# PJLab-ADG/neuralsim

Hardware: NVIDIA H100
Metric: Mrays/sec fwd+bwd (higher is better)
Workload: dtype f16

## Files before the change

### neuralsim_b200/csrc/color_tc.cu

```cuda
#include "fused_tc_common.cuh"
#include "sh_device.cuh"

namespace nsb {

struct ColorNetDev {
    DecoderDevTC dec;
    const __half *R1, *rb1, *R2, *rb2, *R3, *rb3;
    int rw, rin, n_appear;
    float fac[3];
};

constexpr int XW = 64;
constexpr int kTileBytes = kTile * XW * 2;
constexpr int kChunk = kTile * 16;

__host__ __device__ inline int ref_col(int k, int n_appear, int nh) {
    if (k < 32) return k < nh ? 22 + k : -1;
    if (k < 35) return k - 32;
    if (k < 51) return 3 + (k - 35);
    if (k < 54) return 19 + (k - 51);
    if (k < 54 + n_appear) return 22 + nh + (k - 54);
    return -1;
}

// ... 388 lines not shown
        __syncthreads();
        if (tid == 0 && tile + gridDim.x < n_tiles) {
            tc::fence_async_smem();
            fetch(tile + gridDim.x);
        }
#pragma unroll
        for (int h = 0; h < 2; ++h)
#pragma unroll
            for (int r = 0; r < 2; ++r) {
                const int64_t row = tile * kTile + h * 64 + tc::frag_row(r);
                if (row < n) {
#pragma unroll
                    for (int c = 0; c < NF / 8; ++c)
                        *reinterpret_cast<float2 *>(dh_out + row * NF + tc::frag_col(c)) = make_float2(dh[h][4 * c + 2 * r], dh[h][4 * c + 2 * r + 1]);
                    if constexpr (kAppear) *reinterpret_cast<float2 *>(da_out + row * 8 + tc::frag_col(0)) = make_float2(da[h][2 * r], da[h][2 * r + 1]);
                    if constexpr (kRays) {
#pragma unroll
                        for (int c = 0; c < 3; ++c)
                            *reinterpret_cast<float2 *>(xv_out + row * 24 + tc::frag_col(c)) = make_float2(dxv[h][4 * c + 2 * r], dxv[h][4 * c + 2 * r + 1]);
                    }
                }
            }
    }
    if (!first_tile) {
#pragma unroll
        for (int r = 0; r < 2; ++r) {
            const int row = tc::frag_row(r);
            if (row >= net.rw) continue;
#pragma unroll
            for (int c = 0; c < NE / 8; ++c)
#pragma unroll
                for (int j = 0; j < 2; ++j) {
                    const int col = tc::frag_col(c) + j;
                    const float a = xa[4 * c + 2 * r + j], b = xb[4 * c + 2 * r + j];
                    if (col < XW) {
                        if (col < net.rw) atomicAdd(dR2 + row * net.rw + col, a);
                        const int rc = ref_col(col, net.n_appear, net.dec.nh);
                        if (rc >= 0) atomicAdd(dR1 + row * net.rin + rc, b);
                    } else if (col == XW) {
                        atomicAdd(drb2 + row, a);
                        atomicAdd(drb1 + row, b);
                    }
                }
#pragma unroll
            for (int j = 0; j < 2; ++j) {
                const int col = tc::frag_col(0) + j;
                if (col >= 1 && col <= 3) atomicAdd(dR3 + (col - 1) * net.rw + row, x3[2 * r + j]);
            }
        }
        if (tid < 3) atomicAdd(drb3 + tid, sdb3[tid]);
    }
}

template <bool kXGrad>
__global__ void __launch_bounds__(kTile, kColorBwdCtasPerSM)
k_color_sdf_bwd(const PLMeta m, const __half *__restrict__ grid, const ColorNetDev net, const PointSrc ps, const uint8_t *__restrict__ Zt,
                const uint8_t *__restrict__ Xt, const float *__restrict__ g_nab, const float *__restrict__ g_sdf, const float *__restrict__ dh_r,
                int64_t n, int max_level, float *__restrict__ d_grid, float *__restrict__ d_W1, float *__restrict__ d_b1, float *__restrict__ d_W2,
                float *__restrict__ d_b2, const int64_t *__restrict__ n_dev, const float *__restrict__ xv_rows,
                const float *__restrict__ view_dirs, float *__restrict__ gx_out) {
    n = eff_n(n, n_dev);
    constexpr int NX = 48;
    extern __shared__ uint8_t dyn_smem[];
    uint8_t *tiles = reinterpret_cast<uint8_t *>((reinterpret_cast<uintptr_t>(dyn_smem) + 1023) & ~uintptr_t(1023));
    uint8_t *sT = tiles;
    uint8_t *sHe = sT + 3 * kTileBytes;
    uint8_t *sGe = sHe + kTile * NX * 2;
    uint8_t *sW1 = sGe + kTile * NX * 2;
    uint8_t *sW1T = sW1 + HW * NF * 2;
    uint8_t *sZ = sW1T + NF * HW * 2;
    constexpr int kS = tc::acc_stride(2 * NF);
    float *stage = reinterpret_cast<float *>(sT);
    static_assert(kTile * kS * 4 <= 3 * kTileBytes, "the staged rows must fit in T");
    __shared__ float sW2[HW], sdsdf[kTile];
    __shared__ float sdb2;
    __shared__ __align__(8) uint64_t mbar_ld;

    const int tid = threadIdx.x, lane = tid & 31;
    stage_W1(net.dec, sW1, tid);
    stage_W1T(net.dec, sW1T, tid);
    stage_decoder_vectors(net.dec, nullptr, sW2, nullptr, tid);
    *reinterpret_cast<uint4 *>(sHe + 4 * kChunk + tid * 16) = make_uint4(0x00003C00u, 0, 0, 0);
    *reinterpret_cast<uint4 *>(sGe + 4 * kChunk + tid * 16) = make_uint4(0x00003C00u, 0, 0, 0);
    *reinterpret_cast<uint4 *>(sHe + 5 * kChunk + tid * 16) = make_uint4(0, 0, 0, 0);
    *reinterpret_cast<uint4 *>(sGe + 5 * kChunk + tid * 16) = make_uint4(0, 0, 0, 0);
    float wacc[NX / 2], vacc[4];
#pragma unroll
    for (int k = 0; k < NX / 2; ++k) wacc[k] = 0.f;
#pragma unroll
    for (int k = 0; k < 4; ++k) vacc[k] = 0.f;
    if (tid == 0) {
        sdb2 = 0.f;
        tc::mbar_init(&mbar_ld, 1);
        tc::fence_mbar_init();
    }
    tc::fence_async_smem();
    __syncthreads();
    const uint32_t t_addr = tc::smem_u32(sT), he_addr = tc::smem_u32(sHe), ge_addr = tc::smem_u32(sGe), w1_addr = tc::smem_u32(sW1),
                   w1t_addr = tc::smem_u32(sW1T);
    const SoftplusK spk(net.dec.beta);
    uint32_t ld_phase = 0;
    bool first_tile = true;

    const int64_t n_tiles = (n + kTile - 1) / kTile;
    auto fetch = [&](int64_t tile) {
        tc::mbar_arrive_expect_tx(&mbar_ld, kTileBytes + 4 * kChunk);
        tc::tma_load_bulk(sZ, Zt + tile * kTileBytes, kTileBytes, &mbar_ld);
        tc::tma_load_bulk(sHe, Xt + tile * kTileBytes, 4 * kChunk, &mbar_ld);
    };
    if (tid == 0 && (int64_t)blockIdx.x < n_tiles) fetch(blockIdx.x);
    for (int64_t tile = blockIdx.x; tile < n_tiles; tile += gridDim.x) {
        const int64_t i = tile * kTile + tid;
        const bool valid = i < n;
        float xn[3], xs[3];
        int64_t ray;
        load_point(ps, ps.x == nullptr, i, valid, xn, xs, ray);
        float gin[3] = {0.f, 0.f, 0.f};
        if (valid && g_nab) {
#pragma unroll
            for (int d = 0; d < 3; ++d) gin[d] = g_nab[i * 3 + d] * net.fac[d] * 0.5f;
        }
        const float dsdf = (valid && g_sdf) ? g_sdf[i] : 0.f;
        sdsdf[tid] = dsdf;
        tc::mbar_wait(&mbar_ld, ld_phase);
        ld_phase ^= 1;
#pragma unroll 1
        for (int c = 0; c < 8; ++c) {
            float z[8], uu[8];
            unpack8(*reinterpret_cast<const uint4 *>(sZ + c * kChunk + tid * 16), z);
#pragma unroll
            for (int j = 0; j < 8; ++j) {
                float a, s;
                softplus_as(z[j], spk, a, s);
                uu[j] = sW2[c * 8 + j] * s;
            }
            *reinterpret_cast<uint4 *>(sT + kTileBytes + c * kChunk + tid * 16) = tc::pack8_f16(uu);
        }
#pragma unroll 4
        for (uint32_t p = 0; p < 16; ++p) {
            uint32_t packed = 0;
            if (p < m.n_pseudo && (int)m.level[p] <= max_level) {
                float J0[3], J1[3];
                level_jacobian(m, p, xs, grid, J0, J1);
                float a0 = 0.f, a1 = 0.f;
#pragma unroll
                for (int d = 0; d < 3; ++d) { a0 = __fmaf_rn(gin[d], J0[d], a0); a1 = __fmaf_rn(gin[d], J1[d], a1); }
                const __half2 h = __floats2half2_rn(a0, a1);
                packed = *reinterpret_cast<const uint32_t *>(&h);
            }
            *reinterpret_cast<uint32_t *>(sGe + (p >> 2) * kChunk + tid * 16 + (p & 3) * 4) = packed;
        }
        tc::fence_async_smem();
        __syncthreads();
        float gfr[2][NF / 2];
        {
            float du[2][HW / 2];
            tc::mma_m128<64, 0, 0, NF / 16>(du, tc::kmajor(ge_addr, kTile), tc::kmajor(w1_addr, HW), false);
            tc::mma_m128<32, 0, 0, HW / 16>(gfr, tc::kmajor(t_addr + kTileBytes, kTile), tc::kmajor(w1t_addr, NF), false);
#pragma unroll
            for (int h = 0; h < 2; ++h)
#pragma unroll
                for (int r = 0; r < 2; ++r) {
                    const int row = h * 64 + tc::frag_row(r);
                    const float ds = sdsdf[row];
#pragma unroll
                    for (int c = 0; c < HW / 8; ++c) {
                        const int col = tc::frag_col(c);
                        const uint32_t off = tc::pair_off<kTile>(row, col);
                        const float2 z2 = tc::ld_pair_f16(sZ, off);
                        float dz[2], vv[2];
#pragma unroll
                        for (int j = 0; j < 2; ++j) {
                            const float z = j ? z2.y : z2.x;
                            float a, s;
                            softplus_as(z, spk, a, s);
                            const float w2 = sW2[col + j], d = r16(du[h][4 * c + 2 * r + j]);
                            const float curv = (z * spk.k > spk.thr) ? 0.f : spk.beta * s * (1.f - s);
                            dz[j] = d * w2 * curv + ds * w2 * s;
                            vv[j] = d * s + ds * r16(a);
                        }
                        tc::st_pair_f16(sT, off, dz[0], dz[1]);
                        tc::st_pair_f16(sT + 2 * kTileBytes, off, vv[0], vv[1]);
                    }
                }
        }
        tc::fence_async_smem();
        __syncthreads();
        float dhz[2][NF / 2];
        tc::mma_m128<32, 0, 0, HW / 16>(dhz, tc::kmajor(t_addr, kTile), tc::kmajor(w1t_addr, NF), false);
        tc::mma_m64<NX, 1, 1, kTile / 16>(wacc, tc::mnmajor(t_addr, kTile), tc::mnmajor(he_addr, kTile), true);
        tc::mma_m64<NF, 1, 1, kTile / 16>(*reinterpret_cast<float(*)[NF / 2]>(wacc), tc::mnmajor(t_addr + kTileBytes, kTile), tc::mnmajor(ge_addr, kTile), true);
        tc::mma_m64<8, 1, 1, kTile / 16>(vacc, tc::mnmajor(t_addr + 2 * kTileBytes, kTile), tc::mnmajor(ge_addr + 4 * kChunk, kTile), true);
        first_tile = false;
        const float dsum = warp_sum(dsdf);
        if (lane == 0 && dsum != 0.f) atomicAdd(&sdb2, dsum);
        __syncthreads();
        if (tid == 0 && tile + gridDim.x < n_tiles) {
            tc::fence_async_smem();
            fetch(tile + gridDim.x);
        }
        tc::frag_store<NF>(gfr, stage, kS, 0);
        tc::frag_store<NF>(dhz, stage, kS, NF);
        __syncthreads();
        float gx[3] = {0.f, 0.f, 0.f};
#pragma unroll 1
        for (uint32_t g4 = 0; g4 * 4 < m.n_pseudo; ++g4) {
            float gg[8], hz[8];
            tc::acc_ld8(stage, kS, tid, g4 * 8, gg);
            tc::acc_ld8(stage, kS, tid, NF + g4 * 8, hz);
            if (valid && dh_r) {
                const float4 r0 = *reinterpret_cast<const float4 *>(dh_r + i * NF + g4 * 8), r1 = *reinterpret_cast<const float4 *>(dh_r + i * NF + g4 * 8 + 4);
                hz[0] += r0.x; hz[1] += r0.y; hz[2] += r0.z; hz[3] += r0.w; hz[4] += r1.x; hz[5] += r1.y; hz[6] += r1.z; hz[7] += r1.w;
            }
#pragma unroll
            for (uint32_t q = 0; q < 4; ++q) {
                const uint32_t p = g4 * 4 + q;
                if (p >= m.n_pseudo || (int)m.level[p] > max_level) continue;
                uint32_t cell[8];
                float w[8], fr[3], sc[3], ua[8], ub[8];
                level_cells3(m, p, xs, cell, w, fr, sc);
                const float g0 = valid ? r16(gg[2 * q]) : 0.f, g1 = valid ? r16(gg[2 * q + 1]) : 0.f;
                const float h0 = valid ? hz[2 * q] : 0.f, h1 = valid ? hz[2 * q + 1] : 0.f;
                if constexpr (kXGrad) level_input_grad(m, p, grid, cell, fr, sc, h0, h1, gx);
#pragma unroll
                for (int c = 0; c < 8; ++c) {
                    float wsum = 0.f;
#pragma unroll
                    for (int gd = 0; gd < 3; ++gd) {
                        float ww = __fmul_rn(sc[gd], gin[gd]);
#pragma unroll
                        for (int d = 0; d < 3; ++d) {
                            if (d == gd) continue;
                            ww = __fmul_rn(ww, (c & (1 << d)) ? fr[d] : __fsub_rn(1.f, fr[d]));
                        }
                        wsum += (c & (1 << gd)) ? ww : -ww;
                    }
                    ua[c] = g0 * wsum + h0 * w[c];
                    ub[c] = g1 * wsum + h1 * w[c];
                }
                if (warp_merge_updates(cell_key3(m, p, xs), valid, ua, ub, lane)) {
                    float2 *gp = level_grad_ptr(m, p, d_grid);
#pragma unroll
                    for (int c = 0; c < 8; ++c) red_add2(gp + cell[c], ua[c], ub[c]);
                }
            }
        }
        if constexpr (kXGrad) {
            if (valid) {
                float g[3], gv[3] = {0.f, 0.f, 0.f};
#pragma unroll
                for (int d = 0; d < 3; ++d) g[d] = input_grad_to_net(gx[d]);
                if (xv_rows) {
                    const float *xr = xv_rows + i * 24;
#pragma unroll
                    for (int d = 0; d < 3; ++d) g[d] = __fadd_rn(g[d], xr[d]);
                    float jx[16], jy[16], jz[16];
                    sh_jacobian(view_dirs[ray * 3], view_dirs[ray * 3 + 1], view_dirs[ray * 3 + 2], 4, jx, jy, jz);
#pragma unroll
                    for (int c = 0; c < 16; ++c) {
                        const float dsh = xr[3 + c];
                        gv[0] = fmaf(dsh, jx[c], gv[0]); gv[1] = fmaf(dsh, jy[c], gv[1]); gv[2] = fmaf(dsh, jz[c], gv[2]);
                    }
                }
                const float tt = ps.t[i];
                float4 *o = reinterpret_cast<float4 *>(gx_out + i * 12);
                o[0] = make_float4(g[0], g[1], g[2], __fmul_rn(tt, g[0]));
                o[1] = make_float4(__fmul_rn(tt, g[1]), __fmul_rn(tt, g[2]), gv[0], gv[1]);
                o[2] = make_float4(gv[2], 0.f, 0.f, 0.f);
            }
        }
        __syncthreads();
    }
    if (!first_tile) {
#pragma unroll
        for (int r = 0; r < 2; ++r) {
            const int row = tc::frag_row(r);
            if (row >= net.dec.width) continue;
#pragma unroll
            for (int c = 0; c <= NF / 8; ++c)
#pragma unroll
                for (int j = 0; j < 2; ++j) {
                    const int col = tc::frag_col(c) + j;
                    if (col < net.dec.nh) atomicAdd(d_W1 + row * net.dec.nh + col, wacc[4 * c + 2 * r + j]);
                    else if (col == NF) atomicAdd(d_b1 + row, wacc[4 * c + 2 * r + j]);
                }
            if (tc::frag_col(0) == 0) atomicAdd(d_W2 + row, vacc[2 * r]);
        }
        if (tid == 0) atomicAdd(d_b2, sdb2);
    }
}

}

using namespace nsb;

namespace {
int make_net(const nsb_color_net *c, const nsb_lotd_meta *meta, PLMeta *m, ColorNetDev *d, const char *who, bool radiance) {
    const nsb_sdf_decoder dec{c->W1, c->b1, c->W2, c->b2, c->width, c->beta};
    if (int rc = make_decoder(meta, &dec, m, &d->dec, who)) return rc;
    if (radiance || c->rad_width != 0) {
        NSB_REQUIRE(c->rad_width >= 1 && c->rad_width <= 64, "%s: radiance width must be <= 64", who);
        NSB_REQUIRE(c->n_appear >= 0 && c->n_appear <= 8 && c->rad_in == 22 + d->dec.nh + c->n_appear,
                    "%s: radiance input must be [x(3), SH deg 4 (16), n(3), h(2L = %d), h_appear(<=8)]", who, d->dec.nh);
    } else {
        NSB_REQUIRE(!c->R1 && !c->rb1 && !c->R2 && !c->rb2 && !c->R3 && !c->rb3, "%s: rad_width 0 (no radiance net) needs NULL radiance pointers", who);
    }
    d->R1 = (const __half *)c->R1; d->rb1 = (const __half *)c->rb1; d->R2 = (const __half *)c->R2; d->rb2 = (const __half *)c->rb2;
    d->R3 = (const __half *)c->R3; d->rb3 = (const __half *)c->rb3;
    d->rw = c->rad_width; d->rin = c->rad_in; d->n_appear = c->n_appear;
    for (int k = 0; k < 3; ++k) d->fac[k] = c->nablas_scale[k];
    return 0;
}
}

static int64_t n_tiles(int64_t n) { return (n + kTile - 1) / kTile; }

extern "C" int64_t nsb_color_tile_bytes(int64_t n) { return n_tiles(n) * (int64_t)kTileBytes; }

extern "C" int nsb_fused_color_fwd(const nsb_lotd_meta *meta, const void *params_half, const nsb_color_net *net, const float *x, const float *rays_o,
                                   const float *rays_d, const int64_t *ridx, const float *t, const float *view_dirs, const float *h_appear,
                                   int64_t n, int32_t max_level, float *sdf, float *nablas, float *rgb, float *x_out, void *act_z, void *act_x,
                                   void *act_y1, void *act_y2, const nsb_occ_collect *collect, void *stream) {
    const DevCounts dn = take_counts();
    if (n == 0) return 0;
    const bool rad = rgb != nullptr;
// ... 25 lines not shown
    constexpr int kSmem = 2 * kTileBytes + 2 * HW * NF * 2 + 2 * XW * XW * 2 + kTile * tc::acc_stride(64) * 4 + 1024;
    opt_in_smem(k_color_fwd<true>, kSmem);
    k_color_fwd<true><<<persistent_grid(n_tiles(n), 2), kTile, kSmem, (cudaStream_t)stream>>>(m, (const __half *)params_half, d, ps, view_dirs, h_appear, n,
                                                                                             ml, sdf, nablas, rgb, x_out, (uint8_t *)act_z,
                                                                                             (uint8_t *)act_x, (uint8_t *)act_y1, (uint8_t *)act_y2,
                                                                                             occ_collect_of(collect), dn.a);
    return check_launch("nsb_fused_color_fwd");
}

template <bool kAppear, bool kRays>
static int color_bwd(const char *who, const nsb_lotd_meta *meta, const void *params_half, const nsb_color_net *net, const float *x, const float *rays_o,
                     const float *rays_d, const int64_t *ridx, const float *t, int64_t n, int32_t max_level, const void *act_z, const void *act_x,
                     const void *act_y1, const void *act_y2, const float *rgb, const float *g_sdf, const float *g_nablas, const float *g_rgb,
                     float *dh_scratch, float *d_grid, float *d_W1, float *d_b1, float *d_W2, float *d_b2, float *d_R1, float *d_rb1, float *d_R2,
                     float *d_rb2, float *d_R3, float *d_rb3, const float *view_dirs, float *ha_scratch, const int64_t *ray_map, float *d_h_appear,
                     float *ray_scratch, float *d_rays_o, float *d_rays_d, float *d_view_dirs, void *stream) {
    const DevCounts dn = take_counts();
    if (n == 0) return 0;
    NSB_REQUIRE(meta && params_half && net && act_z && act_x, "%s: NULL argument", who);
    NSB_REQUIRE(d_grid && d_W1 && d_b1 && d_W2 && d_b2, "%s: NULL gradient buffer", who);
    if (g_rgb) {
        NSB_REQUIRE(act_y1 && act_y2 && rgb && dh_scratch, "%s: NULL argument (g_rgb given)", who);
        NSB_REQUIRE(d_R1 && d_rb1 && d_R2 && d_rb2 && d_R3 && d_rb3, "%s: NULL radiance gradient buffer (g_rgb given)", who);
    }
    if (kAppear) NSB_REQUIRE(g_rgb && ha_scratch && d_h_appear, "%s: needs g_rgb, ha_scratch and d_h_appear", who);
    if (kRays) {
        NSB_REQUIRE(!x && rays_o && rays_d && t && ray_scratch, "%s: ray gradients need the points as rays (x NULL, rays_o, rays_d, t) and ray_scratch", who);
        NSB_REQUIRE(!g_rgb || view_dirs, "%s: ray gradients with g_rgb need view_dirs", who);
    }
    NSB_REQUIRE(x || (rays_o && rays_d && t), "%s: need x or (rays_o, rays_d, t)", who);
    PLMeta m;
    ColorNetDev d;
    if (int rc = make_net(net, meta, &m, &d, who, g_rgb != nullptr)) return rc;
    if (kAppear) NSB_REQUIRE(d.n_appear >= 1, "%s: the net has no appearance channels", who);
    cudaStream_t s = (cudaStream_t)stream;
    const float *dh = nullptr;
    float *xv_rows = (kRays && g_rgb) ? ray_scratch + n * 12 : nullptr;
    if (g_rgb) {
        constexpr int kSmemR = 3 * kTileBytes + 2 * kTile * 80 * 2 + XW * XW * 2 + NF * XW * 2 + (kAppear || kRays ? 8 * XW * 2 : 0) +
                               (kRays ? NF * XW * 2 : 0) + 1024;
        opt_in_smem(k_color_rad_bwd<kAppear, kRays>, kSmemR);
        if (int rc = require_ctas_per_sm(k_color_rad_bwd<kAppear, kRays>, kTile, kSmemR, kColorBwdCtasPerSM, "nsb_fused_color_bwd(radiance)")) return rc;
        k_color_rad_bwd<kAppear, kRays><<<persistent_grid(n_tiles(n), kColorBwdCtasPerSM), kTile, kSmemR, s>>>(
            d, (const uint8_t *)act_x, (const uint8_t *)act_y1, (const uint8_t *)act_y2, rgb, g_rgb, n, dh_scratch, d_R1, d_rb1, d_R2, d_rb2, d_R3, d_rb3,
            dn.a, ha_scratch, xv_rows);
        if (int rc = check_launch("nsb_fused_color_bwd(radiance)")) return rc;
        dh = dh_scratch;
        if (kAppear) {
            k_ray_row_sum<8><<<row_sum_blocks(n), 256, 0, s>>>(ha_scratch, ridx, nullptr, n, d.n_appear, ray_map,
                                                                RowSumOut{{d_h_appear, nullptr, nullptr}, d.n_appear}, dn.a);
            if (int rc = check_launch("nsb_fused_color_bwd(code sum)")) return rc;
        }
    }
    constexpr int kSmemS = 3 * kTileBytes + 2 * kTile * 48 * 2 + 2 * HW * NF * 2 + kTileBytes + 1024;
    opt_in_smem(k_color_sdf_bwd<kRays>, kSmemS);
    if (int rc = require_ctas_per_sm(k_color_sdf_bwd<kRays>, kTile, kSmemS, kColorBwdCtasPerSM, "nsb_fused_color_bwd(sdf)")) return rc;
    const PointSrc ps{x, rays_o, rays_d, t, ridx};
    k_color_sdf_bwd<kRays><<<persistent_grid(n_tiles(n), kColorBwdCtasPerSM), kTile, kSmemS, s>>>(
        m, (const __half *)params_half, d, ps, (const uint8_t *)act_z, (const uint8_t *)act_x, g_nablas, g_sdf, dh, n, max_level < 0 ? -1 : max_level,
        d_grid, d_W1, d_b1, d_W2, d_b2, dn.a, xv_rows, view_dirs, ray_scratch);
    if (int rc = check_launch("nsb_fused_color_bwd(sdf)")) return rc;
    if (kRays) {
        k_ray_row_sum<12><<<row_sum_blocks(n), 256, 0, s>>>(ray_scratch, ridx, nullptr, n, 9, ray_map, RowSumOut{{d_rays_o, d_rays_d, d_view_dirs}, 3},
                                                             dn.a);
        return check_launch("nsb_fused_color_bwd(ray sum)");
    }
    return 0;
}

extern "C" int nsb_fused_color_bwd(const nsb_lotd_meta *meta, const void *params_half, const nsb_color_net *net, const float *x, const float *rays_o,
                                   const float *rays_d, const int64_t *ridx, const float *t, int64_t n, int32_t max_level, const void *act_z,
                                   const void *act_x, const void *act_y1, const void *act_y2, const float *rgb, const float *g_sdf,
                                   const float *g_nablas, const float *g_rgb, float *dh_scratch, float *d_grid, float *d_W1, float *d_b1,
                                   float *d_W2, float *d_b2, float *d_R1, float *d_rb1, float *d_R2, float *d_rb2, float *d_R3, float *d_rb3,
                                   void *stream) {
    return color_bwd<false, false>("nsb_fused_color_bwd", meta, params_half, net, x, rays_o, rays_d, ridx, t, n, max_level, act_z, act_x, act_y1, act_y2,
                                   rgb, g_sdf, g_nablas, g_rgb, dh_scratch, d_grid, d_W1, d_b1, d_W2, d_b2, d_R1, d_rb1, d_R2, d_rb2, d_R3, d_rb3, nullptr,
                                   nullptr, nullptr, nullptr, nullptr, nullptr, nullptr, nullptr, stream);
}

extern "C" int nsb_fused_color_bwd_appear(const nsb_lotd_meta *meta, const void *params_half, const nsb_color_net *net, const float *x,
                                          const float *rays_o, const float *rays_d, const int64_t *ridx, const float *t, int64_t n, int32_t max_level,
                                          const void *act_z, const void *act_x, const void *act_y1, const void *act_y2, const float *rgb,
                                          const float *g_sdf, const float *g_nablas, const float *g_rgb, float *dh_scratch, float *d_grid,
                                          float *d_W1, float *d_b1, float *d_W2, float *d_b2, float *d_R1, float *d_rb1, float *d_R2, float *d_rb2,
                                          float *d_R3, float *d_rb3, float *ha_scratch, const int64_t *ray_map, float *d_h_appear, void *stream) {
    return color_bwd<true, false>("nsb_fused_color_bwd_appear", meta, params_half, net, x, rays_o, rays_d, ridx, t, n, max_level, act_z, act_x, act_y1,
                                  act_y2, rgb, g_sdf, g_nablas, g_rgb, dh_scratch, d_grid, d_W1, d_b1, d_W2, d_b2, d_R1, d_rb1, d_R2, d_rb2, d_R3, d_rb3,
                                  nullptr, ha_scratch, ray_map, d_h_appear, nullptr, nullptr, nullptr, nullptr, stream);
}

extern "C" int nsb_fused_color_bwd_grads(const nsb_lotd_meta *meta, const void *params_half, const nsb_color_net *net, const float *x,
                                         const float *rays_o, const float *rays_d, const int64_t *ridx, const float *t, int64_t n, int32_t max_level,
                                         const void *act_z, const void *act_x, const void *act_y1, const void *act_y2, const float *rgb,
                                         const float *g_sdf, const float *g_nablas, const float *g_rgb, float *dh_scratch, float *d_grid,
                                         float *d_W1, float *d_b1, float *d_W2, float *d_b2, float *d_R1, float *d_rb1, float *d_R2, float *d_rb2,
                                         float *d_R3, float *d_rb3, const float *view_dirs, float *ha_scratch, const int64_t *ray_map,
                                         float *d_h_appear, float *ray_scratch, float *d_rays_o, float *d_rays_d, float *d_view_dirs, void *stream) {
    const char *who = "nsb_fused_color_bwd_grads";
    const bool appear = d_h_appear != nullptr, rays = d_rays_o || d_rays_d || d_view_dirs;
#define NSB_COLOR_BWD(A, R)                                                                                                                       \
    color_bwd<A, R>(who, meta, params_half, net, x, rays_o, rays_d, ridx, t, n, max_level, act_z, act_x, act_y1, act_y2, rgb, g_sdf, g_nablas, g_rgb, \
                    dh_scratch, d_grid, d_W1, d_b1, d_W2, d_b2, d_R1, d_rb1, d_R2, d_rb2, d_R3, d_rb3, view_dirs, ha_scratch, ray_map, d_h_appear,    \
                    ray_scratch, d_rays_o, d_rays_d, d_view_dirs, stream)
    const int rc = appear ? (rays ? NSB_COLOR_BWD(true, true) : NSB_COLOR_BWD(true, false))
                          : (rays ? NSB_COLOR_BWD(false, true) : NSB_COLOR_BWD(false, false));
#undef NSB_COLOR_BWD
    return rc;
}
```

### neuralsim_b200/csrc/tc_util.cuh

```cuda
#pragma once
#include "nsb_common.cuh"

namespace nsb {
namespace tc {

__device__ __forceinline__ uint32_t smem_u32(const void *p) { return (uint32_t)__cvta_generic_to_shared(p); }

__device__ __forceinline__ uint64_t make_desc(uint32_t smem_addr, uint32_t lbo_bytes, uint32_t sbo_bytes) {
    uint64_t d = 0;
    d |= (uint64_t)((smem_addr >> 4) & 0x3FFF);
    d |= (uint64_t)((lbo_bytes >> 4) & 0x3FFF) << 16;
    d |= (uint64_t)((sbo_bytes >> 4) & 0x3FFF) << 32;
    return d;
}

struct Operand {
    uint32_t addr, lbo, sbo, kstep;
};
__device__ __forceinline__ Operand kmajor(uint32_t addr, int rows) { return Operand{addr, (uint32_t)rows * 16, 128, (uint32_t)rows * 32}; }
__device__ __forceinline__ Operand mnmajor(uint32_t addr, int rows) { return Operand{addr, 128, (uint32_t)rows * 16, 256}; }

template <int N, int TA, int TB>
struct Wgmma;
template <int TA, int TB>
// ... 138 lines not shown
                d[h][4 * c + 2 * i] = v.x;
                d[h][4 * c + 2 * i + 1] = v.y;
            }
}
template <int N, int TA, int TB, int KSTEPS>
__device__ __forceinline__ void mma_to_rows(float *acc, int stride, int col0, const Operand &a, const Operand &b, bool accumulate) {
    float d[2][N / 2];
    if (accumulate) frag_load<N>(d, acc, stride, col0);
    else {
#pragma unroll
        for (int h = 0; h < 2; ++h)
#pragma unroll
            for (int i = 0; i < N / 2; ++i) d[h][i] = 0.f;
    }
    mma_m128<N, TA, TB, KSTEPS>(d, a, b, accumulate);
    frag_store<N>(d, acc, stride, col0);
}

__device__ __forceinline__ void acc_ld8(const float *acc, int stride, int row, int col, float (&v)[8]) {
    const float4 a = *reinterpret_cast<const float4 *>(acc + row * stride + col), b = *reinterpret_cast<const float4 *>(acc + row * stride + col + 4);
    v[0] = a.x; v[1] = a.y; v[2] = a.z; v[3] = a.w; v[4] = b.x; v[5] = b.y; v[6] = b.z; v[7] = b.w;
}

__device__ __forceinline__ void mbar_init(uint64_t *bar, uint32_t count) {
    asm volatile("mbarrier.init.shared::cta.b64 [%0], %1;" ::"r"(smem_u32(bar)), "r"(count) : "memory");
}
__device__ __forceinline__ void mbar_arrive(uint64_t *bar) {
    asm volatile("mbarrier.arrive.shared::cta.b64 _, [%0];" ::"r"(smem_u32(bar)) : "memory");
}
__device__ __forceinline__ void mbar_wait(uint64_t *bar, uint32_t parity) {
    asm volatile(
        "{\n\t.reg .pred p;\n\tWAIT_%=:\n\t"
        "mbarrier.try_wait.parity.shared::cta.b64 p, [%0], %1;\n\t"
        "@p bra DONE_%=;\n\tbra WAIT_%=;\n\tDONE_%=:\n\t}\n" ::"r"(smem_u32(bar)),
        "r"(parity)
        : "memory");
}

__device__ __forceinline__ void mbar_arrive_expect_tx(uint64_t *bar, uint32_t bytes) {
    asm volatile("mbarrier.arrive.expect_tx.shared::cta.b64 _, [%0], %1;" ::"r"(smem_u32(bar)), "r"(bytes) : "memory");
}
__device__ __forceinline__ void tma_load_bulk(void *smem_dst, const void *gmem_src, uint32_t bytes, uint64_t *bar) {
    uint64_t pol;
    asm volatile("createpolicy.fractional.L2::evict_first.b64 %0, 1.0;" : "=l"(pol));
    asm volatile("cp.async.bulk.shared::cluster.global.mbarrier::complete_tx::bytes.L2::cache_hint [%0], [%1], %2, [%3], %4;"
                 ::"r"(smem_u32(smem_dst)), "l"(gmem_src), "r"(bytes), "r"(smem_u32(bar)), "l"(pol)
                 : "memory");
}

template <int N>
__device__ __forceinline__ void setmaxnreg_dec() { asm volatile("setmaxnreg.dec.sync.aligned.u32 %0;" ::"n"(N)); }
template <int N>
__device__ __forceinline__ void setmaxnreg_inc() { asm volatile("setmaxnreg.inc.sync.aligned.u32 %0;" ::"n"(N)); }

__device__ __forceinline__ void fence_async_smem() { asm volatile("fence.proxy.async.shared::cta;" ::: "memory"); }
__device__ __forceinline__ void fence_mbar_init() { asm volatile("fence.mbarrier_init.release.cluster;" ::: "memory"); }

__device__ __forceinline__ uint4 pack8_f16(const float (&v)[8]) {
    __half2 h0 = __floats2half2_rn(v[0], v[1]), h1 = __floats2half2_rn(v[2], v[3]);
    __half2 h2 = __floats2half2_rn(v[4], v[5]), h3 = __floats2half2_rn(v[6], v[7]);
    uint4 q;
    q.x = *reinterpret_cast<uint32_t *>(&h0); q.y = *reinterpret_cast<uint32_t *>(&h1);
    q.z = *reinterpret_cast<uint32_t *>(&h2); q.w = *reinterpret_cast<uint32_t *>(&h3);
    return q;
}

template <int R, int K>
__device__ __forceinline__ void store_row_f16(uint8_t *tile, int r, const float *vals) {
#pragma unroll
    for (int c = 0; c < K / 8; ++c) {
        __half2 h0 = __floats2half2_rn(vals[c * 8 + 0], vals[c * 8 + 1]);
        __half2 h1 = __floats2half2_rn(vals[c * 8 + 2], vals[c * 8 + 3]);
        __half2 h2 = __floats2half2_rn(vals[c * 8 + 4], vals[c * 8 + 5]);
        __half2 h3 = __floats2half2_rn(vals[c * 8 + 6], vals[c * 8 + 7]);
        uint4 q;
        q.x = *reinterpret_cast<uint32_t *>(&h0);
        q.y = *reinterpret_cast<uint32_t *>(&h1);
        q.z = *reinterpret_cast<uint32_t *>(&h2);
        q.w = *reinterpret_cast<uint32_t *>(&h3);
        *reinterpret_cast<uint4 *>(tile + c * (R * 16) + r * 16) = q;
    }
}

}
}
```

Measured before the change: 32.71.

## Warp-specialize color SDF backward into producer, MMA consumer, and scatter roles

Restructures the SDF color backward kernel into a persistent, warp-specialized pipeline. Two producer warpgroups TMA-load Z/X tiles and compute the Jacobian gather into a double-buffered input ring. One consumer warpgroup runs the wgmma chain and also recomputes the upstream softplus derivative inline instead of in a separate pre-pass. Two scatter warpgroups consume a double-buffered output ring to do the hash-grid atomic scatter and input gradients. Registers are rebalanced with setmaxnreg and the launch drops to one CTA per SM with 640 threads. This trades multi-CTA occupancy and extra shared memory for overlap of gather, MMA and scatter phases, and it adds a host check that fails if the compiled register count differs from the assumed split.

```diff
diff --git a/neuralsim_b200/csrc/color_tc.cu b/neuralsim_b200/csrc/color_tc.cu
--- a/neuralsim_b200/csrc/color_tc.cu
+++ b/neuralsim_b200/csrc/color_tc.cu
@@ -464,111 +464,280 @@
     }
 }
 
+constexpr int kCsbProducers = 2, kCsbScatterSets = 2, kCsbInSlots = 2, kCsbOutSlots = 2;
+constexpr int kCsbThreads = kTile * (1 + kCsbProducers + kCsbScatterSets);
+constexpr int kCsbLaunchRegs = (65536 / kCsbThreads) & ~7;
+constexpr int kCsbConsumerRegs = 152, kCsbProducerRegs = 56, kCsbScatterRegs = 104;
+constexpr int kCsbGatherU = 1;
+static_assert(kTile * (kCsbConsumerRegs + kCsbProducers * kCsbProducerRegs + kCsbScatterSets * kCsbScatterRegs) <= kCsbThreads * kCsbLaunchRegs, "register split");
+template <int N>
+__device__ __forceinline__ void csb_set_regs() {
+    static_assert(N % 8 == 0 && N >= 24 && N <= 256, "setmaxnreg range");
+    if constexpr (N > kCsbLaunchRegs) tc::setmaxnreg_inc<N>();
+    else if constexpr (N < kCsbLaunchRegs) tc::setmaxnreg_dec<N>();
+}
+constexpr int kCsbNX = 48;
+constexpr int kCsbHS = tc::acc_stride(NF);
+constexpr int kCsbGS = 40;
+constexpr int kCsbInBytes = kTileBytes + 2 * kTile * kCsbNX * 2 + kTile * 4;
+constexpr int kCsbOutBytes = kTile * kCsbHS * 4 + kTile * kCsbGS * 2;
+constexpr int kCsbSmem = kCsbInSlots * kCsbInBytes + 3 * kTileBytes + kCsbOutSlots * kCsbOutBytes + 2 * HW * NF * 2 + 128;
+
+struct CsbRing {
+    uint8_t *in;
+    uint8_t *out;
+    uint64_t *in_full, *in_empty;
+    uint64_t *out_full, *out_empty;
+    int *end;
+    int64_t *out_tile;
+};
+template <bool kFull>
+__device__ __forceinline__ uint32_t ring_parity(uint32_t j, int slots) { return ((j / (uint32_t)slots) & 1u) ^ (kFull ? 0u : 1u); }
+
+__device__ __forceinline__ uint8_t *csb_he(uint8_t *slot) { return slot + kTileBytes; }
+__device__ __forceinline__ uint8_t *csb_ge(uint8_t *slot) { return slot + kTileBytes + kTile * kCsbNX * 2; }
+__device__ __forceinline__ float *csb_dsdf(uint8_t *slot) { return reinterpret_cast<float *>(slot + kTileBytes + 2 * kTile * kCsbNX * 2); }
+
+__device__ __forceinline__ void csb_produce(const PLMeta &m, const __half *__restrict__ grid, const ColorNetDev &net, const PointSrc &ps,
+                                            const uint8_t *__restrict__ Zt, const uint8_t *__restrict__ Xt, const float *__restrict__ g_nab,
+                                            const float *__restrict__ g_sdf, int64_t n, int max_level, const CsbRing &ring, int set, int r) {
+    const int64_t n_tiles = (n + kTile - 1) / kTile;
+    const uint32_t my_tiles = n_tiles > (int64_t)blockIdx.x ? (uint32_t)((n_tiles - blockIdx.x + gridDim.x - 1) / gridDim.x) : 0u;
+    for (uint32_t j = set; j < my_tiles; j += kCsbProducers) {
+        const int64_t tile = blockIdx.x + (int64_t)j * gridDim.x;
+        const uint32_t s = j % kCsbInSlots;
+        uint8_t *slot = ring.in + s * kCsbInBytes;
+        tc::mbar_wait(&ring.in_empty[s], ring_parity<false>(j, kCsbInSlots));
+        if (r == 0) {
+            tc::fence_async_smem();
+            tc::mbar_arrive_expect_tx(&ring.in_full[s], kTileBytes + 4 * kChunk);
+            tc::tma_load_bulk(slot, Zt + tile * kTileBytes, kTileBytes, &ring.in_full[s]);
+            tc::tma_load_bulk(csb_he(slot), Xt + tile * kTileBytes, 4 * kChunk, &ring.in_full[s]);
+        }
+        const int64_t i = tile * kTile + r;
+        const bool valid = i < n;
+        float xs[3];
+        load_point(ps, ps.x == nullptr, i, valid, xs);
+        float gin[3] = {0.f, 0.f, 0.f};
+        if (valid && g_nab) {
+#pragma unroll
+            for (int d = 0; d < 3; ++d) gin[d] = g_nab[i * 3 + d] * net.fac[d] * 0.5f;
+        }
+        csb_dsdf(slot)[r] = (valid && g_sdf) ? g_sdf[i] : 0.f;
+        uint8_t *sGe = csb_ge(slot);
+#pragma unroll kCsbGatherU
+        for (uint32_t p = 0; p < 16; ++p) {
+            uint32_t packed = 0;
+            if (p < m.n_pseudo && (int)m.level[p] <= max_level) {
+                float J0[3], J1[3];
+                level_jacobian(m, p, xs, grid, J0, J1);
+                float a0 = 0.f, a1 = 0.f;
+#pragma unroll
+                for (int d = 0; d < 3; ++d) { a0 = __fmaf_rn(gin[d], J0[d], a0); a1 = __fmaf_rn(gin[d], J1[d], a1); }
+                const __half2 h = __floats2half2_rn(a0, a1);
+                packed = *reinterpret_cast<const uint32_t *>(&h);
+            }
+            *reinterpret_cast<uint32_t *>(sGe + (p >> 2) * kChunk + r * 16 + (p & 3) * 4) = packed;
+        }
+        tc::fence_async_smem();
+        tc::mbar_arrive(&ring.in_full[s]);
+    }
+    if (my_tiles % kCsbProducers == (uint32_t)set) {
+        const uint32_t s = my_tiles % kCsbInSlots;
+        tc::mbar_wait(&ring.in_empty[s], ring_parity<false>(my_tiles, kCsbInSlots));
+        if (r == 0) {
+            ring.end[s] = 1;
+            tc::mbar_arrive(&ring.in_full[s]);
+        }
+        tc::mbar_arrive(&ring.in_full[s]);
+    }
+}
+
 template <bool kXGrad>
-__global__ void __launch_bounds__(kTile, kColorBwdCtasPerSM)
+__global__ void __launch_bounds__(kCsbThreads, 1)
 k_color_sdf_bwd(const PLMeta m, const __half *__restrict__ grid, const ColorNetDev net, const PointSrc ps, const uint8_t *__restrict__ Zt,
                 const uint8_t *__restrict__ Xt, const float *__restrict__ g_nab, const float *__restrict__ g_sdf, const float *__restrict__ dh_r,
                 int64_t n, int max_level, float *__restrict__ d_grid, float *__restrict__ d_W1, float *__restrict__ d_b1, float *__restrict__ d_W2,
                 float *__restrict__ d_b2, const int64_t *__restrict__ n_dev, const float *__restrict__ xv_rows,
                 const float *__restrict__ view_dirs, float *__restrict__ gx_out) {
     n = eff_n(n, n_dev);
-    constexpr int NX = 48;
+    constexpr int NX = kCsbNX;
     extern __shared__ uint8_t dyn_smem[];
-    uint8_t *tiles = reinterpret_cast<uint8_t *>((reinterpret_cast<uintptr_t>(dyn_smem) + 1023) & ~uintptr_t(1023));
-    uint8_t *sT = tiles;
-    uint8_t *sHe = sT + 3 * kTileBytes;
-    uint8_t *sGe = sHe + kTile * NX * 2;
-    uint8_t *sW1 = sGe + kTile * NX * 2;
+    uint8_t *base = reinterpret_cast<uint8_t *>((reinterpret_cast<uintptr_t>(dyn_smem) + 127) & ~uintptr_t(127));
+    CsbRing ring;
+    ring.in = base;
+    uint8_t *sT = ring.in + kCsbInSlots * kCsbInBytes;
+    ring.out = sT + 3 * kTileBytes;
+    uint8_t *sW1 = ring.out + kCsbOutSlots * kCsbOutBytes;
     uint8_t *sW1T = sW1 + HW * NF * 2;
-    uint8_t *sZ = sW1T + NF * HW * 2;
-    constexpr int kS = tc::acc_stride(2 * NF);
-    float *stage = reinterpret_cast<float *>(sT);
-    static_assert(kTile * kS * 4 <= 3 * kTileBytes, "the staged rows must fit in T");
-    __shared__ float sW2[HW], sdsdf[kTile];
+    __shared__ float sW2[HW];
     __shared__ float sdb2;
-    __shared__ __align__(8) uint64_t mbar_ld;
-
-    const int tid = threadIdx.x, lane = tid & 31;
-    stage_W1(net.dec, sW1, tid);
-    stage_W1T(net.dec, sW1T, tid);
-    stage_decoder_vectors(net.dec, nullptr, sW2, nullptr, tid);
-    *reinterpret_cast<uint4 *>(sHe + 4 * kChunk + tid * 16) = make_uint4(0x00003C00u, 0, 0, 0);
-    *reinterpret_cast<uint4 *>(sGe + 4 * kChunk + tid * 16) = make_uint4(0x00003C00u, 0, 0, 0);
-    *reinterpret_cast<uint4 *>(sHe + 5 * kChunk + tid * 16) = make_uint4(0, 0, 0, 0);
-    *reinterpret_cast<uint4 *>(sGe + 5 * kChunk + tid * 16) = make_uint4(0, 0, 0, 0);
-    float wacc[NX / 2], vacc[4];
-#pragma unroll
-    for (int k = 0; k < NX / 2; ++k) wacc[k] = 0.f;
-#pragma unroll
-    for (int k = 0; k < 4; ++k) vacc[k] = 0.f;
+    __shared__ __align__(8) uint64_t bars[2 * kCsbInSlots + 2 * kCsbOutSlots];
+    __shared__ int end_flags[kCsbInSlots];
+    __shared__ int64_t out_tiles[kCsbOutSlots];
+    ring.in_full = bars;
+    ring.in_empty = bars + kCsbInSlots;
+    ring.out_full = bars + 2 * kCsbInSlots;
+    ring.out_empty = ring.out_full + kCsbOutSlots;
+    ring.end = end_flags;
+    ring.out_tile = out_tiles;
+
+    const int tid = threadIdx.x, lane = tid & 31, wg = tid / kTile;
+    if (wg == 0) {
+        stage_W1(net.dec, sW1, tid);
+        stage_W1T(net.dec, sW1T, tid);
+        stage_decoder_vectors(net.dec, nullptr, sW2, nullptr, tid);
+#pragma unroll
+        for (int s = 0; s < kCsbInSlots; ++s) {
+            uint8_t *slot = ring.in + s * kCsbInBytes;
+            *reinterpret_cast<uint4 *>(csb_he(slot) + 4 * kChunk + tid * 16) = make_uint4(0x00003C00u, 0, 0, 0);
+            *reinterpret_cast<uint4 *>(csb_ge(slot) + 4 * kChunk + tid * 16) = make_uint4(0x00003C00u, 0, 0, 0);
+            *reinterpret_cast<uint4 *>(csb_he(slot) + 5 * kChunk + tid * 16) = make_uint4(0, 0, 0, 0);
+            *reinterpret_cast<uint4 *>(csb_ge(slot) + 5 * kChunk + tid * 16) = make_uint4(0, 0, 0, 0);
+        }
+    }
     if (tid == 0) {
         sdb2 = 0.f;
-        tc::mbar_init(&mbar_ld, 1);
-        tc::fence_mbar_init();
-    }
+        for (int s = 0; s < kCsbInSlots; ++s) {
+            tc::mbar_init(&ring.in_full[s], kTile + 1);
+            tc::mbar_init(&ring.in_empty[s], kTile);
+            ring.end[s] = 0;
+        }
+        for (int o = 0; o < kCsbOutSlots; ++o) {
+            tc::mbar_init(&ring.out_full[o], kTile);
+            tc::mbar_init(&ring.out_empty[o], kTile);
+        }
+    }
+    tc::fence_mbar_init();
     tc::fence_async_smem();
     __syncthreads();
-    const uint32_t t_addr = tc::smem_u32(sT), he_addr = tc::smem_u32(sHe), ge_addr = tc::smem_u32(sGe), w1_addr = tc::smem_u32(sW1),
-                   w1t_addr = tc::smem_u32(sW1T);
+
+    if (wg >= 1 && wg <= kCsbProducers) {
+        csb_set_regs<kCsbProducerRegs>();
+        csb_produce(m, grid, net, ps, Zt, Xt, g_nab, g_sdf, n, max_level, ring, wg - 1, tid - wg * kTile);
+        return;
+    }
+    if (wg > kCsbProducers) {
+        csb_set_regs<kCsbScatterRegs>();
+        const int set = wg - 1 - kCsbProducers, r = tid - wg * kTile;
+        for (uint32_t j = set;; j += kCsbScatterSets) {
+            const uint32_t o = j % kCsbOutSlots;
+            tc::mbar_wait(&ring.out_full[o], ring_parity<true>(j, kCsbOutSlots));
+            const int64_t tile = ring.out_tile[o];
+            if (tile < 0) break;
+            const uint8_t *slot = ring.out + o * kCsbOutBytes;
+            const float *hrows = reinterpret_cast<const float *>(slot);
+            const uint8_t *grow = slot + kTile * kCsbHS * 4 + r * (kCsbGS * 2);
+            const int64_t i = tile * kTile + r;
+            const bool valid = i < n;
+            float xn[3], xs[3];
+            int64_t ray;
+            load_point(ps, ps.x == nullptr, i, valid, xn, xs, ray);
+            float gin[3] = {0.f, 0.f, 0.f};
+            if (valid && g_nab) {
+#pragma unroll
+                for (int d = 0; d < 3; ++d) gin[d] = g_nab[i * 3 + d] * net.fac[d] * 0.5f;
+            }
+            float gx[3] = {0.f, 0.f, 0.f};
+#pragma unroll 1
+            for (uint32_t g4 = 0; g4 * 4 < m.n_pseudo; ++g4) {
+                float gg[8], hz[8];
+                unpack8(*reinterpret_cast<const uint4 *>(grow + g4 * 16), gg);
+                tc::acc_ld8(hrows, kCsbHS, r, g4 * 8, hz);
+                if (valid && dh_r) {
+                    const float4 r0 = *reinterpret_cast<const float4 *>(dh_r + i * NF + g4 * 8), r1 = *reinterpret_cast<const float4 *>(dh_r + i * NF + g4 * 8 + 4);
+                    hz[0] += r0.x; hz[1] += r0.y; hz[2] += r0.z; hz[3] += r0.w; hz[4] += r1.x; hz[5] += r1.y; hz[6] += r1.z; hz[7] += r1.w;
+                }
+#pragma unroll
+                for (uint32_t q = 0; q < 4; ++q) {
+                    const uint32_t p = g4 * 4 + q;
+                    if (p >= m.n_pseudo || (int)m.level[p] > max_level) continue;
+                    uint32_t cell[8];
+                    float w[8], fr[3], sc[3], ua[8], ub[8];
+                    level_cells3(m, p, xs, cell, w, fr, sc);
+                    const float g0 = valid ? gg[2 * q] : 0.f, g1 = valid ? gg[2 * q + 1] : 0.f;
+                    const float h0 = valid ? hz[2 * q] : 0.f, h1 = valid ? hz[2 * q + 1] : 0.f;
+                    if constexpr (kXGrad) level_input_grad(m, p, grid, cell, fr, sc, h0, h1, gx);
+#pragma unroll
+                    for (int c = 0; c < 8; ++c) {
+                        float wsum = 0.f;
+#pragma unroll
+                        for (int gd = 0; gd < 3; ++gd) {
+                            float ww = __fmul_rn(sc[gd], gin[gd]);
+#pragma unroll
+                            for (int d = 0; d < 3; ++d) {
+                                if (d == gd) continue;
+                                ww = __fmul_rn(ww, (c & (1 << d)) ? fr[d] : __fsub_rn(1.f, fr[d]));
+                            }
+                            wsum += (c & (1 << gd)) ? ww : -ww;
+                        }
+                        ua[c] = g0 * wsum + h0 * w[c];
+                        ub[c] = g1 * wsum + h1 * w[c];
+                    }
+                    if (warp_merge_updates(cell_key3(m, p, xs), valid, ua, ub, lane)) {
+                        float2 *gp = level_grad_ptr(m, p, d_grid);
+#pragma unroll
+                        for (int c = 0; c < 8; ++c) red_add2(gp + cell[c], ua[c], ub[c]);
+                    }
+                }
+            }
+            tc::mbar_arrive(&ring.out_empty[o]);
+            if constexpr (kXGrad) {
+                if (valid) {
+                    float g[3], gv[3] = {0.f, 0.f, 0.f};
+#pragma unroll
+                    for (int d = 0; d < 3; ++d) g[d] = input_grad_to_net(gx[d]);
+                    if (xv_rows) {
+                        const float *xr = xv_rows + i * 24;
+#pragma unroll
+                        for (int d = 0; d < 3; ++d) g[d] = __fadd_rn(g[d], xr[d]);
+                        float jx[16], jy[16], jz[16];
+                        sh_jacobian(view_dirs[ray * 3], view_dirs[ray * 3 + 1], view_dirs[ray * 3 + 2], 4, jx, jy, jz);
+#pragma unroll
+                        for (int c = 0; c < 16; ++c) {
+                            const float dsh = xr[3 + c];
+                            gv[0] = fmaf(dsh, jx[c], gv[0]); gv[1] = fmaf(dsh, jy[c], gv[1]); gv[2] = fmaf(dsh, jz[c], gv[2]);
+                        }
+                    }
+                    const float tt = ps.t[i];
+                    float4 *ov = reinterpret_cast<float4 *>(gx_out + i * 12);
+                    ov[0] = make_float4(g[0], g[1], g[2], __fmul_rn(tt, g[0]));
+                    ov[1] = make_float4(__fmul_rn(tt, g[1]), __fmul_rn(tt, g[2]), gv[0], gv[1]);
+                    ov[2] = make_float4(gv[2], 0.f, 0.f, 0.f);
+                }
+            }
+        }
+        return;
+    }
+
+    csb_set_regs<kCsbConsumerRegs>();
+    const uint32_t t_addr = tc::smem_u32(sT), w1_addr = tc::smem_u32(sW1), w1t_addr = tc::smem_u32(sW1T);
     const SoftplusK spk(net.dec.beta);
-    uint32_t ld_phase = 0;
+    float wacc[NX / 2], vacc[4];
+#pragma unroll
+    for (int k = 0; k < NX / 2; ++k) wacc[k] = 0.f;
+#pragma unroll
+    for (int k = 0; k < 4; ++k) vacc[k] = 0.f;
     bool first_tile = true;
-
-    const int64_t n_tiles = (n + kTile - 1) / kTile;
-    auto fetch = [&](int64_t tile) {
-        tc::mbar_arrive_expect_tx(&mbar_ld, kTileBytes + 4 * kChunk);
-        tc::tma_load_bulk(sZ, Zt + tile * kTileBytes, kTileBytes, &mbar_ld);
-        tc::tma_load_bulk(sHe, Xt + tile * kTileBytes, 4 * kChunk, &mbar_ld);
-    };
-    if (tid == 0 && (int64_t)blockIdx.x < n_tiles) fetch(blockIdx.x);
-    for (int64_t tile = blockIdx.x; tile < n_tiles; tile += gridDim.x) {
-        const int64_t i = tile * kTile + tid;
-        const bool valid = i < n;
-        float xn[3], xs[3];
-        int64_t ray;
-        load_point(ps, ps.x == nullptr, i, valid, xn, xs, ray);
-        float gin[3] = {0.f, 0.f, 0.f};
-        if (valid && g_nab) {
-#pragma unroll
-            for (int d = 0; d < 3; ++d) gin[d] = g_nab[i * 3 + d] * net.fac[d] * 0.5f;
-        }
-        const float dsdf = (valid && g_sdf) ? g_sdf[i] : 0.f;
-        sdsdf[tid] = dsdf;
-        tc::mbar_wait(&mbar_ld, ld_phase);
-        ld_phase ^= 1;
-#pragma unroll 1
-        for (int c = 0; c < 8; ++c) {
-            float z[8], uu[8];
-            unpack8(*reinterpret_cast<const uint4 *>(sZ + c * kChunk + tid * 16), z);
-#pragma unroll
-            for (int j = 0; j < 8; ++j) {
-                float a, s;
-                softplus_as(z[j], spk, a, s);
-                uu[j] = sW2[c * 8 + j] * s;
-            }
-            *reinterpret_cast<uint4 *>(sT + kTileBytes + c * kChunk + tid * 16) = tc::pack8_f16(uu);
-        }
-#pragma unroll 4
-        for (uint32_t p = 0; p < 16; ++p) {
-            uint32_t packed = 0;
-            if (p < m.n_pseudo && (int)m.level[p] <= max_level) {
-                float J0[3], J1[3];
-                level_jacobian(m, p, xs, grid, J0, J1);
-                float a0 = 0.f, a1 = 0.f;
-#pragma unroll
-                for (int d = 0; d < 3; ++d) { a0 = __fmaf_rn(gin[d], J0[d], a0); a1 = __fmaf_rn(gin[d], J1[d], a1); }
-                const __half2 h = __floats2half2_rn(a0, a1);
-                packed = *reinterpret_cast<const uint32_t *>(&h);
-            }
-            *reinterpret_cast<uint32_t *>(sGe + (p >> 2) * kChunk + tid * 16 + (p & 3) * 4) = packed;
-        }
-        tc::fence_async_smem();
-        __syncthreads();
-        float gfr[2][NF / 2];
+    for (uint32_t j = 0;; ++j) {
+        const uint32_t s = j % kCsbInSlots;
+        tc::mbar_wait(&ring.in_full[s], ring_parity<true>(j, kCsbInSlots));
+        if (ring.end[s]) {
+            for (uint32_t e = j; e < j + kCsbScatterSets; ++e) {
+                const uint32_t o = e % kCsbOutSlots;
+                tc::mbar_wait(&ring.out_empty[o], ring_parity<false>(e, kCsbOutSlots));
+                if (tid == 0) ring.out_tile[o] = -1;
+                tc::mbar_arrive(&ring.out_full[o]);
+            }
+            break;
+        }
+        uint8_t *slot = ring.in + s * kCsbInBytes;
+        const uint8_t *sZ = slot;
+        const float *sdsdf = csb_dsdf(slot);
+        const uint32_t he_addr = tc::smem_u32(csb_he(slot)), ge_addr = tc::smem_u32(csb_ge(slot));
         {
             float du[2][HW / 2];
             tc::mma_m128<64, 0, 0, NF / 16>(du, tc::kmajor(ge_addr, kTile), tc::kmajor(w1_addr, HW), false);
-            tc::mma_m128<32, 0, 0, HW / 16>(gfr, tc::kmajor(t_addr + kTileBytes, kTile), tc::kmajor(w1t_addr, NF), false);
 #pragma unroll
             for (int h = 0; h < 2; ++h)
 #pragma unroll
@@ -580,109 +749,55 @@
                         const int col = tc::frag_col(c);
                         const uint32_t off = tc::pair_off<kTile>(row, col);
                         const float2 z2 = tc::ld_pair_f16(sZ, off);
-                        float dz[2], vv[2];
-#pragma unroll
-                        for (int j = 0; j < 2; ++j) {
-                            const float z = j ? z2.y : z2.x;
-                            float a, s;
-                            softplus_as(z, spk, a, s);
-                            const float w2 = sW2[col + j], d = r16(du[h][4 * c + 2 * r + j]);
-                            const float curv = (z * spk.k > spk.thr) ? 0.f : spk.beta * s * (1.f - s);
-                            dz[j] = d * w2 * curv + ds * w2 * s;
-                            vv[j] = d * s + ds * r16(a);
+                        float dz[2], uu[2], vv[2];
+#pragma unroll
+                        for (int jj = 0; jj < 2; ++jj) {
+                            const float z = jj ? z2.y : z2.x;
+                            float a, sg;
+                            softplus_as(z, spk, a, sg);
+                            const float w2 = sW2[col + jj], d = r16(du[h][4 * c + 2 * r + jj]);
+                            const float curv = (z * spk.k > spk.thr) ? 0.f : spk.beta * sg * (1.f - sg);
+                            uu[jj] = w2 * sg;
+                            dz[jj] = d * w2 * curv + ds * w2 * sg;
+                            vv[jj] = d * sg + ds * r16(a);
                         }
                         tc::st_pair_f16(sT, off, dz[0], dz[1]);
+                        tc::st_pair_f16(sT + kTileBytes, off, uu[0], uu[1]);
                         tc::st_pair_f16(sT + 2 * kTileBytes, off, vv[0], vv[1]);
                     }
                 }
         }
         tc::fence_async_smem();
-        __syncthreads();
-        float dhz[2][NF / 2];
+        tc::named_barrier(1, kTile);
+        float gfr[2][NF / 2], dhz[2][NF / 2];
+        tc::mma_m128<32, 0, 0, HW / 16>(gfr, tc::kmajor(t_addr + kTileBytes, kTile), tc::kmajor(w1t_addr, NF), false);
         tc::mma_m128<32, 0, 0, HW / 16>(dhz, tc::kmajor(t_addr, kTile), tc::kmajor(w1t_addr, NF), false);
         tc::mma_m64<NX, 1, 1, kTile / 16>(wacc, tc::mnmajor(t_addr, kTile), tc::mnmajor(he_addr, kTile), true);
         tc::mma_m64<NF, 1, 1, kTile / 16>(*reinterpret_cast<float(*)[NF / 2]>(wacc), tc::mnmajor(t_addr + kTileBytes, kTile), tc::mnmajor(ge_addr, kTile), true);
         tc::mma_m64<8, 1, 1, kTile / 16>(vacc, tc::mnmajor(t_addr + 2 * kTileBytes, kTile), tc::mnmajor(ge_addr + 4 * kChunk, kTile), true);
         first_tile = false;
-        const float dsum = warp_sum(dsdf);
+        const float dsum = warp_sum(sdsdf[tid]);
         if (lane == 0 && dsum != 0.f) atomicAdd(&sdb2, dsum);
-        __syncthreads();
-        if (tid == 0 && tile + gridDim.x < n_tiles) {
-            tc::fence_async_smem();
-            fetch(tile + gridDim.x);
-        }
-        tc::frag_store<NF>(gfr, stage, kS, 0);
-        tc::frag_store<NF>(dhz, stage, kS, NF);
-        __syncthreads();
-        float gx[3] = {0.f, 0.f, 0.f};
-#pragma unroll 1
-        for (uint32_t g4 = 0; g4 * 4 < m.n_pseudo; ++g4) {
-            float gg[8], hz[8];
-            tc::acc_ld8(stage, kS, tid, g4 * 8, gg);
-            tc::acc_ld8(stage, kS, tid, NF + g4 * 8, hz);
-            if (valid && dh_r) {
-                const float4 r0 = *reinterpret_cast<const float4 *>(dh_r + i * NF + g4 * 8), r1 = *reinterpret_cast<const float4 *>(dh_r + i * NF + g4 * 8 + 4);
-                hz[0] += r0.x; hz[1] += r0.y; hz[2] += r0.z; hz[3] += r0.w; hz[4] += r1.x; hz[5] += r1.y; hz[6] += r1.z; hz[7] += r1.w;
-            }
-#pragma unroll
-            for (uint32_t q = 0; q < 4; ++q) {
-                const uint32_t p = g4 * 4 + q;
-                if (p >= m.n_pseudo || (int)m.level[p] > max_level) continue;
-                uint32_t cell[8];
-                float w[8], fr[3], sc[3], ua[8], ub[8];
-                level_cells3(m, p, xs, cell, w, fr, sc);
-                const float g0 = valid ? r16(gg[2 * q]) : 0.f, g1 = valid ? r16(gg[2 * q + 1]) : 0.f;
-                const float h0 = valid ? hz[2 * q] : 0.f, h1 = valid ? hz[2 * q + 1] : 0.f;
-                if constexpr (kXGrad) level_input_grad(m, p, grid, cell, fr, sc, h0, h1, gx);
-#pragma unroll
-                for (int c = 0; c < 8; ++c) {
-                    float wsum = 0.f;
-#pragma unroll
-                    for (int gd = 0; gd < 3; ++gd) {
-                        float ww = __fmul_rn(sc[gd], gin[gd]);
-#pragma unroll
-                        for (int d = 0; d < 3; ++d) {
-                            if (d == gd) continue;
-                            ww = __fmul_rn(ww, (c & (1 << d)) ? fr[d] : __fsub_rn(1.f, fr[d]));
-                        }
-                        wsum += (c & (1 << gd)) ? ww : -ww;
-                    }
-                    ua[c] = g0 * wsum + h0 * w[c];
-                    ub[c] = g1 * wsum + h1 * w[c];
-                }
-                if (warp_merge_updates(cell_key3(m, p, xs), valid, ua, ub, lane)) {
-                    float2 *gp = level_grad_ptr(m, p, d_grid);
-#pragma unroll
-                    for (int c = 0; c < 8; ++c) red_add2(gp + cell[c], ua[c], ub[c]);
-                }
-            }
-        }
-        if constexpr (kXGrad) {
-            if (valid) {
-                float g[3], gv[3] = {0.f, 0.f, 0.f};
-#pragma unroll
-                for (int d = 0; d < 3; ++d) g[d] = input_grad_to_net(gx[d]);
-                if (xv_rows) {
-                    const float *xr = xv_rows + i * 24;
-#pragma unroll
-                    for (int d = 0; d < 3; ++d) g[d] = __fadd_rn(g[d], xr[d]);
-                    float jx[16], jy[16], jz[16];
-                    sh_jacobian(view_dirs[ray * 3], view_dirs[ray * 3 + 1], view_dirs[ray * 3 + 2], 4, jx, jy, jz);
-#pragma unroll
-                    for (int c = 0; c < 16; ++c) {
-                        const float dsh = xr[3 + c];
-                        gv[0] = fmaf(dsh, jx[c], gv[0]); gv[1] = fmaf(dsh, jy[c], gv[1]); gv[2] = fmaf(dsh, jz[c], gv[2]);
-                    }
-                }
-                const float tt = ps.t[i];
-                float4 *o = reinterpret_cast<float4 *>(gx_out + i * 12);
-                o[0] = make_float4(g[0], g[1], g[2], __fmul_rn(tt, g[0]));
-                o[1] = make_float4(__fmul_rn(tt, g[1]), __fmul_rn(tt, g[2]), gv[0], gv[1]);
-                o[2] = make_float4(gv[2], 0.f, 0.f, 0.f);
-            }
-        }
-        __syncthreads();
-    }
+        tc::mbar_arrive(&ring.in_empty[s]);
+        tc::named_barrier(1, kTile);
+        const uint32_t o = j % kCsbOutSlots;
+        tc::mbar_wait(&ring.out_empty[o], ring_parity<false>(j, kCsbOutSlots));
+        uint8_t *oslot = ring.out + o * kCsbOutBytes;
+        tc::frag_store<NF>(dhz, reinterpret_cast<float *>(oslot), kCsbHS, 0);
+        uint8_t *gst = oslot + kTile * kCsbHS * 4;
+#pragma unroll
+        for (int h = 0; h < 2; ++h)
+#pragma unroll
+            for (int c = 0; c < NF / 8; ++c)
+#pragma unroll
+                for (int r = 0; r < 2; ++r) {
+                    const int row = h * 64 + tc::frag_row(r), col = tc::frag_col(c);
+                    *reinterpret_cast<__half2 *>(gst + row * (kCsbGS * 2) + col * 2) = __floats2half2_rn(gfr[h][4 * c + 2 * r], gfr[h][4 * c + 2 * r + 1]);
+                }
+        if (tid == 0) ring.out_tile[o] = blockIdx.x + (int64_t)j * gridDim.x;
+        tc::mbar_arrive(&ring.out_full[o]);
+    }
+    tc::named_barrier(1, kTile);
     if (!first_tile) {
 #pragma unroll
         for (int r = 0; r < 2; ++r) {
@@ -814,11 +929,19 @@
             if (int rc = check_launch("nsb_fused_color_bwd(code sum)")) return rc;
         }
     }
-    constexpr int kSmemS = 3 * kTileBytes + 2 * kTile * 48 * 2 + 2 * HW * NF * 2 + kTileBytes + 1024;
-    opt_in_smem(k_color_sdf_bwd<kRays>, kSmemS);
-    if (int rc = require_ctas_per_sm(k_color_sdf_bwd<kRays>, kTile, kSmemS, kColorBwdCtasPerSM, "nsb_fused_color_bwd(sdf)")) return rc;
+    opt_in_smem(k_color_sdf_bwd<kRays>, kCsbSmem);
+    if (int rc = require_ctas_per_sm(k_color_sdf_bwd<kRays>, kCsbThreads, kCsbSmem, 1, "nsb_fused_color_bwd(sdf)")) return rc;
+    {
+        static int regs = 0;
+        if (!regs) {
+            cudaFuncAttributes fa{};
+            cudaFuncGetAttributes(&fa, k_color_sdf_bwd<kRays>);
+            regs = fa.numRegs;
+        }
+        NSB_REQUIRE(regs == kCsbLaunchRegs, "nsb_fused_color_bwd(sdf): compiled at %d registers per thread, the role split assumes %d", regs, kCsbLaunchRegs);
+    }
     const PointSrc ps{x, rays_o, rays_d, t, ridx};
-    k_color_sdf_bwd<kRays><<<persistent_grid(n_tiles(n), kColorBwdCtasPerSM), kTile, kSmemS, s>>>(
+    k_color_sdf_bwd<kRays><<<persistent_grid(n_tiles(n), 1), kCsbThreads, kCsbSmem, s>>>(
         m, (const __half *)params_half, d, ps, (const uint8_t *)act_z, (const uint8_t *)act_x, g_nablas, g_sdf, dh, n, max_level < 0 ? -1 : max_level,
         d_grid, d_W1, d_b1, d_W2, d_b2, dn.a, xv_rows, view_dirs, ray_scratch);
     if (int rc = check_launch("nsb_fused_color_bwd(sdf)")) return rc;
diff --git a/neuralsim_b200/csrc/tc_util.cuh b/neuralsim_b200/csrc/tc_util.cuh
--- a/neuralsim_b200/csrc/tc_util.cuh
+++ b/neuralsim_b200/csrc/tc_util.cuh
@@ -214,6 +214,8 @@
 __device__ __forceinline__ void setmaxnreg_dec() { asm volatile("setmaxnreg.dec.sync.aligned.u32 %0;" ::"n"(N)); }
 template <int N>
 __device__ __forceinline__ void setmaxnreg_inc() { asm volatile("setmaxnreg.inc.sync.aligned.u32 %0;" ::"n"(N)); }
+
+__device__ __forceinline__ void named_barrier(int id, int threads) { asm volatile("bar.sync %0, %1;" ::"r"(id), "r"(threads) : "memory"); }
 
 __device__ __forceinline__ void fence_async_smem() { asm volatile("fence.proxy.async.shared::cta;" ::: "memory"); }
 __device__ __forceinline__ void fence_mbar_init() { asm volatile("fence.mbarrier_init.release.cluster;" ::: "memory"); }
```

New measurement: 33.03, median of 6. No clear change (+1.0%).
